# sencheng/CoBeL-RL

Measured on NVIDIA B200. Metric: agent-steps/sec incl. replay, higher is better.
Workload: dtype f64

## Files before the change

### cobel-rl_b200/csrc/dynaq.cu

```cuda
#include "warp_agent.cuh"

namespace {

constexpr int kWarpsPerCta = 4;

struct AgentSmem {
  int q, mr, mx, wm, rm, ptab, draws, vmax, pat, bytes;
  __host__ __device__ AgentSmem(int S, int A, bool plain, bool tables = true, bool sums = false) {
    const bool eps_tab = plain && A <= 4;
    const int SA = tables ? S * A : 0;
    q = 0;
    mr = q + SA * 8;
    wm = mr + SA * 8;
    rm = wm + S * 4;
    mx = rm + S * 4;
    ptab = (mx + SA * 2 + 15) & ~15;
    draws = ptab + (eps_tab ? kEpsTabDoubles * 8 : 0);
    vmax = draws + (plain ? kSmemDraws * 8 : 0);
    pat = vmax + (sums ? S * 8 : 0);
    bytes = sums ? (pat + S + 15) & ~15 : vmax;
  }
};

struct WorldSmem {
  int rew, succ, starts, term, bytes;
  __host__ __device__ WorldSmem(int S, int A, int K) {
    rew = 0;
    succ = rew + S * 8;
    starts = succ + S * A * 4;
    term = starts + K * 4;
    bytes = (term + S + 15) & ~15;
  }
};

template <int A, bool PLAIN, bool HBM = false, bool SUM = false>
__global__ void __launch_bounds__(kWarpsPerCta * 32, HBM ? 1 : 7) dynaq_warp_kernel(const __grid_constant__ CobelDynaQParams p) {
  static_assert(!(PLAIN && HBM), "the HBM path is the generic kernel");
  static_assert(!SUM || (PLAIN && A <= 4), "row summaries go with the tie-pattern table");
  extern __shared__ __align__(16) unsigned char smem[];
  const int S = p.world.n_states, K = p.world.n_starts, SA = S * A;
  const int lane = threadIdx.x & 31, warp = threadIdx.x >> 5;
  const WorldSmem wo(HBM ? 0 : S, A, HBM ? 0 : K);
  constexpr bool kEpsTab = PLAIN && A <= 4;
  const AgentSmem ao(S, A, PLAIN, !HBM, SUM);

  double* rew_s = reinterpret_cast<double*>(smem + wo.rew);
  int32_t* succ_s = reinterpret_cast<int32_t*>(smem + wo.succ);
  int32_t* starts_s = reinterpret_cast<int32_t*>(smem + wo.starts);
  uint8_t* term_s = smem + wo.term;
  if constexpr (!HBM) {
    for (int e = threadIdx.x; e < SA; e += blockDim.x) succ_s[e] = p.world.succ[e];
    for (int e = threadIdx.x; e < S; e += blockDim.x) { rew_s[e] = p.world.reward[e]; term_s[e] = p.world.terminal[e]; }
    for (int e = threadIdx.x; e < K; e += blockDim.x) starts_s[e] = p.world.starts[e];
    __syncthreads();
  }
  auto w_succ = [&](int sa) -> int { if constexpr (HBM) return __ldg(p.world.succ + sa); else return succ_s[sa]; };
  auto w_rew = [&](int x) -> double { if constexpr (HBM) return __ldg(p.world.reward + x); else return rew_s[x]; };
  auto w_term = [&](int x) -> int { if constexpr (HBM) return __ldg(p.world.terminal + x); else return term_s[x]; };
  auto w_start = [&](int k) -> int { if constexpr (HBM) return __ldg(p.world.starts + k); else return starts_s[k]; };

  const int64_t n = (int64_t)blockIdx.x * blockDim.x / 32 + warp;
  if (n >= p.n_agents) return;

  unsigned char* blk = smem + wo.bytes + (size_t)warp * ao.bytes;
  const size_t g0 = (size_t)n * SA;
  double* Q = HBM ? p.Q + g0 : reinterpret_cast<double*>(blk + ao.q);
  double* Mr = HBM ? p.Mr + g0 : reinterpret_cast<double*>(blk + ao.mr);
  uint16_t* Mx = reinterpret_cast<uint16_t*>(blk + ao.mx);
  int32_t* Msg = p.Ms + g0;
  int32_t* Mtg = p.Mt + g0;
  uint32_t* wm = reinterpret_cast<uint32_t*>(blk + ao.wm);
  uint32_t* rm = reinterpret_cast<uint32_t*>(blk + ao.rm);
  auto m_next = [&](int i, int& s2, int& nt) {
    if constexpr (HBM) { s2 = Msg[i]; nt = Mtg[i] ? 1 : 0; }
    else { const uint16_t v = Mx[i]; s2 = v & 0x7FFF; nt = v >> 15; }
  };
  auto m_set = [&](int i, int s2, int nt) {
    if constexpr (HBM) { Msg[i] = s2; Mtg[i] = nt; }
    else Mx[i] = (uint16_t)(s2 | (nt << 15));
  };

  if constexpr (!HBM) {
    for (int e = lane; e < SA; e += 32) {
      Q[e] = p.Q[g0 + e];
      Mr[e] = p.Mr[g0 + e];
      Mx[e] = (uint16_t)(p.Ms[g0 + e] | ((p.Mt[g0 + e] ? 1 : 0) << 15));
    }
  }
  __syncwarp();

  for (int e = lane; e < S; e += 32) { wm[e] = 0; rm[e] = 0; }
  double* V = reinterpret_cast<double*>(blk + ao.vmax);
  uint8_t* P = blk + ao.pat;
  if constexpr (SUM)
    for (int e = lane; e < S; e += 32) refresh_row_summary<A>(Q, V, P, e);
  typename WindowFor<PLAIN>::type win; win.init(p.stream, n, (uint64_t)p.stream.draw_count[n]);
  win.attach(reinterpret_cast<double*>(blk + ao.draws));
  const double lr = p.lr[n], gamma = p.gamma[n], mlr = p.mem_lr[n];
  PolicyTab pt; pt.init(p.policy.kind, p.policy.param[n], lane);
  double* ptab = reinterpret_cast<double*>(blk + ao.ptab);
  if constexpr (kEpsTab) eps_cdf_table_init<A>(ptab, pt, lane);
  const uint8_t* amask = (!PLAIN && p.action_mask) ? p.action_mask + n * p.mask_agent_stride : nullptr;
  const int B = PLAIN ? 32 : p.batch;
  const bool learn = PLAIN || p.learn != 0;
  const bool step_replay = PLAIN || (learn && !p.no_replay && !p.episodic_replay);
  const bool trial_replay = !PLAIN && learn && !p.no_replay && p.episodic_replay;
  const CobelTrace& tr = p.trace;
  int64_t nsteps = 0, nrep = 0, ncalls = 0;
  int flags = 0;

  auto replay = [&]() {
    for (int b0 = 0; b0 < B; b0 += 32) {
      const int nb = B - b0 < 32 ? B - b0 : 32;
      win.ensure(nb, lane);
      const bool active = lane < nb;
      const double u = win.peek(active ? lane : 0);
      win.advance(nb);
      int rs = 0, ra = 0, rs2 = 0, rnt = 0;
      double rr = 0.0;
      if (active) {
        const int i = draw_integer(u, SA);
        rs = i / A; ra = i - rs * A;
        rr = Mr[i];
        m_next(i, rs2, rnt);
        if (!PLAIN && tr.replay_idx) {
          if (nrep + lane < tr.replay_cap) tr.replay_idx[n * tr.replay_cap + nrep + lane] = i;
          else flags |= COBEL_FLAG_TRACE_OVERFLOW;
        }
      }
      td_batch_level_parallel<A>(Q, wm, rm, S, lane, active, rs, ra, rr, rs2, rnt, lr, gamma);
      nrep += nb;
    }
    if (!PLAIN && tr.replay_len && lane == 0) {
      if (ncalls < tr.replay_calls_cap) tr.replay_len[n * tr.replay_calls_cap + ncalls] = B;
      else flags |= COBEL_FLAG_TRACE_OVERFLOW;
    }
    ++ncalls;
  };

  for (int trial = 0; trial < p.trials; ++trial) {
    win.ensure(3 + (step_replay && B <= 32 ? B : 0), lane);
    int s = w_start(draw_integer(win.next(), K));
    double treward = 0.0;
    int step = 0;
    if constexpr (PLAIN) {
      for (;; ++step) {
        win.ensure(34, lane);
        const int i = draw_integer(win.peek(1 + lane), SA);
        double rr = Mr[i];
        int rs2, rnt;
        m_next(i, rs2, rnt);
        int a;
        if constexpr (SUM) {
          a = select_action_eps_pattern<A>(P[s], ptab, win.next(), lane);
        } else {
          double row[A];
          load_row<A>(Q + s * A, row);
          if constexpr (kEpsTab) a = select_action_eps_tab<A>(row, ptab, win.next(), lane);
          else a = select_action_warp<A, COBEL_POLICY_EPS_GREEDY>(row, (1u << A) - 1u, pt, win.next(), lane);
        }
        const int sa = s * A + a;
        const int s2 = w_succ(sa);
        const double r = w_rew(s2);
        const int end = w_term(s2);
        const int nt = 1 - end;
        const double m0 = Mr[sa];
        const double m1 = xadd(m0, xmul(mlr, xsub(r, m0)));
        double row2[A];
        if constexpr (!SUM) load_row<A>(Q + s2 * A, row2);
        const double q = Q[sa];
        const double g = nt ? gamma : 0.0;
        double td = xadd(r, xmul(g, SUM ? V[s2] : row_max<A>(row2)));
        td = xsub(td, q);
        const double qn = xadd(q, xmul(lr, td));
        if (i == sa) { rr = m1; rs2 = s2; rnt = nt; }
        const int rs = i / A, ra = i - rs * A;
        __syncwarp();
        if (lane == 0) {
          Mr[sa] = m1;
          m_set(sa, s2, nt);
          Q[sa] = qn;
          if (SUM && __double_as_longlong(qn) != __double_as_longlong(q)) refresh_row_summary<A>(Q, V, P, s);
        }
        __syncwarp();
        td_batch_level_parallel<A, SUM>(Q, wm, rm, S, lane, true, rs, ra, rr, rs2, rnt, lr, gamma, nullptr, nullptr, V, P);
        win.advance(32);
        ++nsteps;
        treward = xadd(treward, r);
        if (end || step + 1 == p.steps) break;
        s = s2;
      }
    } else for (;; ++step) {
      win.ensure(2 + (step_replay && B <= 32 ? B : 0), lane);
      double row[A];
      load_row<A>(Q + s * A, row);
      uint32_t mask = (1u << A) - 1u;
      if (amask) {
        mask = 0;
#pragma unroll
        for (int a = 0; a < A; ++a) mask |= (amask[s * A + a] ? 1u : 0u) << a;
      }
      const int a = select_action_warp<A>(row, mask, pt, win.next(), lane);
      const int s2 = p.world.tp_off ? stochastic_successor(p.world, s * A + a, win.next()) : w_succ(s * A + a);
      const double r = w_rew(s2);
      const int end = w_term(s2);
      const int nt = 1 - end;
      if (tr.step_sa && lane == 0) {
        if (nsteps < tr.step_cap) { tr.step_sa[n * tr.step_cap + nsteps] = s * A + a; if (tr.step_next) tr.step_next[n * tr.step_cap + nsteps] = s2; }
        else flags |= COBEL_FLAG_TRACE_OVERFLOW;
      }
      ++nsteps;
      if (learn) {
        const double m0 = Mr[s * A + a];
        const double m1 = xadd(m0, xmul(mlr, xsub(r, m0)));
        double row2[A];
        load_row<A>(Q + s2 * A, row2);
        const double q = Q[s * A + a];
        const double g = nt ? gamma : 0.0;
        double td = xadd(r, xmul(g, row_max<A>(row2)));
        td = xsub(td, q);
        const double qn = xadd(q, xmul(lr, td));
        if (tr.step_td && lane == 0) {
          if (nsteps <= tr.step_cap) tr.step_td[n * tr.step_cap + nsteps - 1] = td;
          else flags |= COBEL_FLAG_TRACE_OVERFLOW;
        }
        __syncwarp();
        if (lane == 0) {
          Mr[s * A + a] = m1;
          m_set(s * A + a, s2, nt);
          Q[s * A + a] = qn;
        }
        __syncwarp();
      }
      s = s2;
      if (step_replay) replay();
      treward = xadd(treward, r);
      if (end || step + 1 == p.steps) break;
    }
    if (lane == 0) {
      tr.trial_steps[n * p.trials + trial] = step;
      tr.trial_reward[n * p.trials + trial] = treward;
    }
    if (trial_replay) replay();
  }

  __syncwarp();
  if (learn && !HBM) {
    for (int e = lane; e < SA; e += 32) {
      p.Q[g0 + e] = Q[e];
      p.Mr[g0 + e] = Mr[e];
      p.Ms[g0 + e] = Mx[e] & 0x7FFF;
      p.Mt[g0 + e] = Mx[e] >> 15;
    }
  }
  flags = __reduce_or_sync(kFull, flags);
  if (lane == 0) {
    p.stream.draw_count[n] = (int64_t)win.position();
    tr.n_steps[n] += nsteps;
    tr.n_replay[n] += PLAIN ? nsteps * 32 : nrep;
    if (tr.flags && flags) tr.flags[n] |= flags;
  }
}


constexpr int kPairWarps = 2;
constexpr int kRing = 128;

struct PairSmem {
  int q, mr, mx, wm, rm, ptab, ring, bytes;
  __host__ __device__ PairSmem(int S, int A) {
    const int SA = S * A;
    q = 0;
    mr = q + SA * 8;
    wm = mr + SA * 8;
    rm = wm + S * 4;
    mx = rm + S * 4;
    ptab = (mx + SA * 2 + 15) & ~15;
    ring = ptab + kEpsTabDoubles * 8;
    bytes = ring + kRing * 8;
  }
};

template <int A>
__global__ void __launch_bounds__(kPairWarps * 32, 14) dynaq_pair_kernel(const __grid_constant__ CobelDynaQParams p) {
  static_assert(A <= 4, "tie-pattern table");
  extern __shared__ __align__(16) unsigned char smem[];
  const int S = p.world.n_states, K = p.world.n_starts, SA = S * A;
  const int lane = threadIdx.x & 31, warp = threadIdx.x >> 5, half = lane >> 4, h = lane & 15;
  const WorldSmem wo(S, A, K);
  const PairSmem ao(S, A);
  double* rew_s = reinterpret_cast<double*>(smem + wo.rew);
  int32_t* succ_s = reinterpret_cast<int32_t*>(smem + wo.succ);
  int32_t* starts_s = reinterpret_cast<int32_t*>(smem + wo.starts);
  uint8_t* term_s = smem + wo.term;
  for (int e = threadIdx.x; e < SA; e += blockDim.x) succ_s[e] = p.world.succ[e];
  for (int e = threadIdx.x; e < S; e += blockDim.x) { rew_s[e] = p.world.reward[e]; term_s[e] = p.world.terminal[e]; }
  for (int e = threadIdx.x; e < K; e += blockDim.x) starts_s[e] = p.world.starts[e];
  __syncthreads();

  const int64_t n = ((int64_t)blockIdx.x * kPairWarps + warp) * 2 + half;
  const bool mine = n < p.n_agents;
  const int64_t nn = mine ? n : p.n_agents - 1;
  unsigned char* blk = smem + wo.bytes + (size_t)(warp * 2 + half) * ao.bytes;
  const size_t g0 = (size_t)nn * SA;
  double* Q = reinterpret_cast<double*>(blk + ao.q);
  double* Mr = reinterpret_cast<double*>(blk + ao.mr);
  uint16_t* Mx = reinterpret_cast<uint16_t*>(blk + ao.mx);
  uint32_t* wm = reinterpret_cast<uint32_t*>(blk + ao.wm);
  uint32_t* rm = reinterpret_cast<uint32_t*>(blk + ao.rm);
  double* ptab = reinterpret_cast<double*>(blk + ao.ptab);
  double* ring = reinterpret_cast<double*>(blk + ao.ring);
  for (int e = h; e < SA; e += 16) {
    Q[e] = mine ? p.Q[g0 + e] : 0.0;
    Mr[e] = mine ? p.Mr[g0 + e] : 0.0;
    Mx[e] = mine ? (uint16_t)(p.Ms[g0 + e] | ((p.Mt[g0 + e] ? 1 : 0) << 15)) : (uint16_t)0;
  }
  for (int e = h; e < S; e += 16) { wm[e] = 0; rm[e] = 0; }
  for (int e = h; e < kRing; e += 16) ring[e] = 0.0;
  const double lr = p.lr[nn], gamma = p.gamma[nn], mlr = p.mem_lr[nn];
  {
    const double eps = p.policy.param[nn];
    const int pat = h & ((1 << A) - 1), k = __popc(pat);
    const double base = xdiv(eps, (double)A);
    const double tie = xdiv(xsub(1.0, eps), (double)(k > 0 ? k : 1));
    const double top = xadd(base, tie), low = xadd(base, 0.0);
    double cdf[A];
    double c = (pat & 1) ? top : low;
    cdf[0] = c;
#pragma unroll
    for (int a = 1; a < A; ++a) { c = xadd(c, (pat >> a & 1) ? top : low); cdf[a] = c; }
    if (c != 1.0) {
#pragma unroll
      for (int a = 0; a < A; ++a) cdf[a] = xdiv(cdf[a], c);
    }
    if (h > 0 && h < (1 << A)) {
#pragma unroll
      for (int a = 0; a < 4; ++a) ptab[pat * 4 + a] = a < A ? cdf[a] : 2.0;
    }
  }
  const uint64_t agent = (uint64_t)(p.stream.agent_id_base + nn);
  const uint32_t key0 = (uint32_t)p.stream.seed, key1 = (uint32_t)(p.stream.seed >> 32);
  const uint64_t pos0 = (uint64_t)p.stream.draw_count[nn];
  uint64_t gblk = (pos0 & ~31ull) >> 1;
  int wr = 0;
  int rd = (int)(pos0 & 31ull);
  int avail = -rd;
  const CobelTrace& tr = p.trace;
  bool live = mine && p.trials > 0;
  bool fresh = true;
  int s = 0, step = 0, trial = 0;
  int nsteps = 0;
  double treward = 0.0;
  __syncwarp();

  while (__any_sync(kFull, live)) {
    for (;;) {
      const bool need = live && avail < 34;
      if (!__any_sync(kFull, need)) break;
      const uint64_t b = gblk + (uint64_t)h;
      uint32_t o[4];
      philox4x32_10((uint32_t)b, (uint32_t)(b >> 32), (uint32_t)agent, (uint32_t)(agent >> 32), key0, key1, o);
      if (need) {
        reinterpret_cast<double2*>(ring)[(wr >> 1) + h] = make_double2(u53(o[0], o[1]), u53(o[2], o[3]));
        gblk += 16; wr = (wr + 32) & (kRing - 1); avail += 32;
      }
    }
    __syncwarp();
    if (fresh) {
      if (live) { s = starts_s[draw_integer(ring[rd], K)]; rd = (rd + 1) & (kRing - 1); --avail; }
      fresh = false; step = 0; treward = 0.0;
    }
    double row[A];
    load_row<A>(Q + s * A, row);
    const double ua = ring[rd];
    int a;
    {
      const double m = row_max<A>(row);
      uint32_t ties = 0;
#pragma unroll
      for (int x = 0; x < A; ++x) ties |= (row[x] == m ? 1u : 0u) << x;
      const double edge = ptab[ties * 4 + (h & 3)];
      const unsigned bal = __ballot_sync(kFull, h < A - 1 && edge <= ua);
      a = __popc((bal >> (half * 16)) & 0xFFFFu);
    }
    const int sa = s * A + a;
    const int s2 = succ_s[sa];
    const double r = rew_s[s2];
    const int end = term_s[s2];
    const int nt = 1 - end;
    {
      const double m0 = Mr[sa];
      const double m1 = xadd(m0, xmul(mlr, xsub(r, m0)));
      double row2[A];
      load_row<A>(Q + s2 * A, row2);
      const double q = Q[sa];
      const double g = nt ? gamma : 0.0;
      double td = xadd(r, xmul(g, row_max<A>(row2)));
      td = xsub(td, q);
      const double qn = xadd(q, xmul(lr, td));
      __syncwarp();
      if (live && h == 0) {
        Mr[sa] = m1;
        Mx[sa] = (uint16_t)(s2 | (nt << 15));
        Q[sa] = qn;
      }
      __syncwarp();
    }
#pragma unroll 1
    for (int b0 = 0; b0 < 32; b0 += 16) {
      const double u = ring[(rd + 1 + b0 + h) & (kRing - 1)];
      const int i = draw_integer(u, SA);
      const int rs = i / A, ra = i - rs * A;
      const double rr = Mr[i];
      const uint16_t v = Mx[i];
      td_batch_level_parallel<A>(Q, wm, rm, S, lane, live, rs, ra, rr, v & 0x7FFF, v >> 15, lr, gamma);
    }
    {
      const bool fin = end || step + 1 == p.steps;
      const double tw = xadd(treward, r);
      if (live && fin && h == 0) {
        tr.trial_steps[n * p.trials + trial] = step;
        tr.trial_reward[n * p.trials + trial] = tw;
      }
      const int adv = live ? 33 : 0;
      rd = (rd + adv) & (kRing - 1); avail -= adv;
      nsteps += live ? 1 : 0;
      treward = tw;
      trial += (live && fin) ? 1 : 0;
      fresh = fin;
      step = step + 1;
      s = s2;
      live = live && trial < p.trials;
    }
  }

  __syncwarp();
  if (mine) {
    for (int e = h; e < SA; e += 16) {
      p.Q[g0 + e] = Q[e];
      p.Mr[g0 + e] = Mr[e];
      p.Ms[g0 + e] = Mx[e] & 0x7FFF;
      p.Mt[g0 + e] = Mx[e] >> 15;
    }
    if (h == 0) {
      p.stream.draw_count[n] = (int64_t)(gblk * 2) - (int64_t)avail;
      tr.n_steps[n] += nsteps;
      tr.n_replay[n] += (int64_t)nsteps * 32;
    }
  }
}

template <int A>
int launch(const CobelDynaQParams& p, cudaStream_t st) {
  const int S = p.world.n_states, K = p.world.n_starts;
  const WorldSmem wo(S, A, K);
  const bool plain = !p.action_mask && !p.world.tp_off && !p.trace.step_sa && !p.trace.step_td && !p.trace.replay_idx &&
                     !p.trace.replay_len &&
                     p.policy.kind == COBEL_POLICY_EPS_GREEDY && p.learn && !p.no_replay && !p.episodic_replay &&
                     p.batch == 32 && !p.stream.user_stream;
  const AgentSmem ao(S, A, plain);
  const size_t sm = (size_t)wo.bytes + (size_t)kWarpsPerCta * ao.bytes;
  const unsigned grid = (unsigned)((p.n_agents + kWarpsPerCta - 1) / kWarpsPerCta);
  if (sm > kMaxSmem) {
    const AgentSmem go(S, A, false, false);
    int warps = kWarpsPerCta;
    while (warps > 1 && (size_t)warps * go.bytes > kMaxSmem) warps >>= 1;
    const size_t smg = (size_t)warps * go.bytes;
    COBEL_REQUIRE(smg <= kMaxSmem, COBEL_EUNSUPPORTED,
                  "Dyna-Q: the replay's dependency masks of %d states do not fit in shared memory (%zu bytes)", S, smg);
    return launch_kernel(dynaq_warp_kernel<A, false, true>, (unsigned)((p.n_agents + warps - 1) / warps), warps * 32, smg, st, p);
  }
  if constexpr (A <= 4) {
    const PairSmem po(S, A);
    const size_t smp = (size_t)wo.bytes + (size_t)kPairWarps * 2 * po.bytes;
    static const int n_sm = [] { int d = 0, v = 148; if (cudaGetDevice(&d) == cudaSuccess) cudaDeviceGetAttribute(&v, cudaDevAttrMultiProcessorCount, d); return v; }();
    if (plain && p.n_agents >= (int64_t)2 * 7 * kWarpsPerCta * n_sm && smp <= kMaxSmem && S <= 0x7FFF) {
      const int64_t per_cta = kPairWarps * 2;
      return launch_kernel(dynaq_pair_kernel<A>, (unsigned)((p.n_agents + per_cta - 1) / per_cta), kPairWarps * 32, smp, st, p);
    }
    const size_t sms = (size_t)wo.bytes + (size_t)kWarpsPerCta * AgentSmem(S, A, true, true, true).bytes;
    if (plain && sms <= kMaxSmem)
      return launch_kernel(dynaq_warp_kernel<A, true, false, true>, grid, kWarpsPerCta * 32, sms, st, p);
  }
  return launch_kernel(plain ? dynaq_warp_kernel<A, true> : dynaq_warp_kernel<A, false>, grid, kWarpsPerCta * 32, sm,
                       st, p);
}

}

extern "C" int cobel_dynaq_run(const CobelDynaQParams* pp, void* stream) {
  COBEL_REQUIRE(pp != nullptr, COBEL_EINVAL, "null params");
  const CobelDynaQParams& p = *pp;
  int rc = cobel_validate_common(p.n_agents, p.world, p.stream, p.policy, p.trace, p.trials, p.steps);
  if (rc) return rc;
  COBEL_REQUIRE(p.Q && p.Mr && p.Ms && p.Mt && p.lr && p.gamma && p.mem_lr, COBEL_EINVAL, "agent tables missing");
  COBEL_REQUIRE(p.batch >= 0, COBEL_EINVAL, "batch must be >= 0");
  if (p.trials == 0) return COBEL_OK;
  cudaStream_t st = reinterpret_cast<cudaStream_t>(stream);
  COBEL_DISPATCH_A(p.world.n_actions, return launch<A>(p, st));
}
```

### cobel-rl_b200/csrc/warp_agent.cuh

```cuda
#pragma once
#include "common.cuh"

constexpr unsigned kFull = 0xffffffffu;

COBEL_DEV double shfl_f64(double v, int src) {
  int lo = __double2loint(v), hi = __double2hiint(v);
  lo = __shfl_sync(kFull, lo, src);
  hi = __shfl_sync(kFull, hi, src);
  return __hiloint2double(hi, lo);
}

COBEL_DEV double shfl_f64_up(double v, int delta) {
  int lo = __double2loint(v), hi = __double2hiint(v);
  lo = __shfl_up_sync(kFull, lo, delta);
  hi = __shfl_up_sync(kFull, hi, delta);
  return __hiloint2double(hi, lo);
}

COBEL_DEV double shfl_f64_xor(double v, int m) {
  int lo = __double2loint(v), hi = __double2hiint(v);
  lo = __shfl_xor_sync(kFull, lo, m);
  hi = __shfl_xor_sync(kFull, hi, m);
  return __hiloint2double(hi, lo);
}

template <int A>
COBEL_DEV void load_row(const double* r, double (&v)[A]) {
  if constexpr (A % 2 == 0) {
#pragma unroll
    for (int x = 0; x < A; x += 2) {
      const double2 t = *reinterpret_cast<const double2*>(r + x);
      v[x] = t.x; v[x + 1] = t.y;
    }
  } else {
#pragma unroll
    for (int x = 0; x < A; ++x) v[x] = r[x];
  }
}

COBEL_DEV int stochastic_successor(const CobelWorld& w, int sa, double u) {
  const int lo = __ldg(w.tp_off + sa), hi = __ldg(w.tp_off + sa + 1);
  double tot = 0.0;
  for (int j = lo; j < hi; ++j) tot = xadd(tot, __ldg(w.tp_prob + j));
  double c = 0.0;
  for (int j = lo; j < hi; ++j) {
    c = xadd(c, __ldg(w.tp_prob + j));
    if (xdiv(c, tot) > u) return __ldg(w.tp_next + j);
  }
  return __ldg(w.tp_next + hi - 1);
}

static __device__ __noinline__ double2 philox_pair_shared(uint64_t b, uint64_t agent, uint32_t key0, uint32_t key1) {
  uint32_t o[4];
  philox4x32_10((uint32_t)b, (uint32_t)(b >> 32), (uint32_t)agent, (uint32_t)(agent >> 32), key0, key1, o);
  return make_double2(u53(o[0], o[1]), u53(o[2], o[3]));
}

template <bool MAYBE_USER, bool SMALL_CODE = false>
struct DrawWindowT {
  uint64_t agent;
  uint32_t key0, key1;
  uint64_t base;
  int off;
  int cap;
  double ua, ub;
  const double* user;
  int64_t user_len;

  COBEL_DEV void init(const CobelStream& s, int64_t local_agent, uint64_t k) {
    agent = (uint64_t)(s.agent_id_base + local_agent);
    key0 = (uint32_t)s.seed; key1 = (uint32_t)(s.seed >> 32);
    user = (MAYBE_USER && s.user_stream) ? s.user_stream + local_agent * s.user_stream_len : nullptr;
    user_len = s.user_stream_len;
    base = k; off = 0; cap = 0;
    ua = ub = 0.0;
  }
  COBEL_DEV uint64_t position() const { return base + (uint64_t)off; }
  COBEL_DEV void ensure(int need, int lane) {
    if ((MAYBE_USER && user) || off + need <= cap) return;
    const uint64_t k = base + (uint64_t)off;
    base = k & ~1ull; off = (int)(k & 1ull); cap = 64;
    const uint64_t b = (base >> 1) + lane;
    if constexpr (SMALL_CODE) {
      const double2 d = philox_pair_shared(b, agent, key0, key1);
      ua = d.x; ub = d.y;
    } else {
      uint32_t o[4];
      philox4x32_10((uint32_t)b, (uint32_t)(b >> 32), (uint32_t)agent, (uint32_t)(agent >> 32), key0, key1, o);
      ua = u53(o[0], o[1]); ub = u53(o[2], o[3]);
    }
  }
  COBEL_DEV double peek(int ahead) const {
    if (MAYBE_USER && user) {
      const uint64_t kk = base + (uint64_t)(off + ahead);
      return kk < (uint64_t)user_len ? user[kk] : 0.0;
    }
    const int slot = off + ahead;
    const double a = shfl_f64(ua, slot >> 1), b = shfl_f64(ub, slot >> 1);
    return (slot & 1) ? b : a;
  }
  COBEL_DEV void advance(int n) { off += n; }
  COBEL_DEV double next() { const double u = peek(0); ++off; return u; }
  COBEL_DEV void attach(double*) {}
};
using DrawWindow = DrawWindowT<true>;

constexpr int kSmemDraws = 256;
template <int NDRAWS>
struct SmemDrawWindowT {
  uint64_t agent;
  uint32_t key0, key1;
  uint64_t base;
  int off;
  int cap;
  double* buf;

  COBEL_DEV void attach(double* b) { buf = b; }
  COBEL_DEV void init(const CobelStream& s, int64_t local_agent, uint64_t k) {
    agent = (uint64_t)(s.agent_id_base + local_agent);
    key0 = (uint32_t)s.seed; key1 = (uint32_t)(s.seed >> 32);
    base = k; off = 0; cap = 0;
  }
  COBEL_DEV uint64_t position() const { return base + (uint64_t)off; }
  COBEL_DEV void ensure(int need, int lane) {
    if (off + need <= cap) return;
    const uint64_t k = base + (uint64_t)off;
    base = k & ~1ull; off = (int)(k & 1ull); cap = NDRAWS;
    __syncwarp();
#pragma unroll
    for (int j = 0; j < NDRAWS / 64; ++j) {
      const uint64_t b = (base >> 1) + (uint64_t)(j * 32 + lane);
      uint32_t o[4];
      philox4x32_10((uint32_t)b, (uint32_t)(b >> 32), (uint32_t)agent, (uint32_t)(agent >> 32), key0, key1, o);
      reinterpret_cast<double2*>(buf)[j * 32 + lane] = make_double2(u53(o[0], o[1]), u53(o[2], o[3]));
    }
    __syncwarp();
  }
  COBEL_DEV double peek(int ahead) const { return buf[off + ahead]; }
  COBEL_DEV void advance(int n) { off += n; }
  COBEL_DEV double next() { return buf[off++]; }
};
using SmemDrawWindow = SmemDrawWindowT<kSmemDraws>;
template <bool PLAIN, int NDRAWS = kSmemDraws> struct WindowFor { using type = DrawWindowT<true>; };
template <int NDRAWS> struct WindowFor<true, NDRAWS> { using type = SmemDrawWindowT<NDRAWS>; };

struct PolicyTab {
  int kind;
  double par;
  double q_par;
  double q_om;
  COBEL_DEV void init(int kind_, double par_, int lane) {
    kind = kind_; par = par_;
    q_par = xdiv(par_, (double)(lane + 1));
    q_om = xdiv(xsub(1.0, par_), (double)(lane + 1));
  }
};

template <int A, int KIND = -1>
COBEL_DEV int select_action_warp(const double (&v)[A], uint32_t mask, const PolicyTab& pt, double u, int lane) {
  const int kind = KIND >= 0 ? KIND : pt.kind;
  constexpr uint32_t kAll = (1u << A) - 1u;
  double m;
  int nv = A;
  if (mask == kAll) {
    m = row_max<A>(v);
  } else {
    nv = __popc(mask);
    m = -__longlong_as_double(0x7FF0000000000000ll);
#pragma unroll
    for (int a = 0; a < A; ++a) m = (mask >> a & 1u) ? xmax(m, v[a]) : m;
  }
  double p[A];
  if (kind == COBEL_POLICY_SOFTMAX) {
    double sum = 0.0;
#pragma unroll
    for (int a = 0; a < A; ++a) {
      p[a] = 0.0;
      if (mask >> a & 1u) { p[a] = exp(xmul(xsub(v[a], m), pt.par)); sum = xadd(sum, p[a]); }
    }
    if (A == 8 && mask == kAll) sum = np_sum<A>(p);
#pragma unroll
    for (int a = 0; a < A; ++a)
      if (mask >> a & 1u) p[a] = xdiv(p[a], sum);
  } else {
    uint32_t ties = 0;
#pragma unroll
    for (int a = 0; a < A; ++a) ties |= (v[a] == m ? 1u : 0u) << a;
    ties &= mask;
    const int k = __popc(ties);
    const double tie = shfl_f64(pt.q_om, k - 1);
    if (kind == COBEL_POLICY_EPS_GREEDY) {
      const double base = shfl_f64(pt.q_par, nv - 1);
      const double top = xadd(base, tie), low = xadd(base, 0.0);
#pragma unroll
      for (int a = 0; a < A; ++a)
        p[a] = (mask >> a & 1u) ? ((ties >> a & 1u) ? top : low) : 0.0;
    } else {
      const int d = nv - k > 1 ? nv - k : 1;
      const double expl = shfl_f64(pt.q_par, d - 1);
      const double top = xadd(tie, 0.0), low = xadd(0.0, expl);
#pragma unroll
      for (int a = 0; a < A; ++a)
        p[a] = (mask >> a & 1u) ? ((ties >> a & 1u) ? top : low) : 0.0;
    }
  }
  double c = p[0], mine = p[0];
#pragma unroll
  for (int a = 1; a < A; ++a) { c = xadd(c, p[a]); if (lane == a) mine = c; }
  if (c != 1.0) mine = xdiv(mine, c);
  const bool le = (lane < A - 1) && (mine <= u);
  return __popc(__ballot_sync(kFull, le));
}

constexpr int kEpsTabDoubles = 64;
template <int A>
COBEL_DEV void eps_cdf_table_init(double* tab, const PolicyTab& pt, int lane) {
  static_assert(A <= 4, "tie-pattern table is built for at most 4 actions");
  const int pat = lane & ((1 << A) - 1);
  const int k = __popc(pat);
  const double base = shfl_f64(pt.q_par, A - 1);
  const double tie = shfl_f64(pt.q_om, k > 0 ? k - 1 : 0);
  const double top = xadd(base, tie), low = xadd(base, 0.0);
  double cdf[A];
  double c = (pat & 1) ? top : low;
  cdf[0] = c;
#pragma unroll
  for (int a = 1; a < A; ++a) { c = xadd(c, (pat >> a & 1) ? top : low); cdf[a] = c; }
  if (c != 1.0) {
#pragma unroll
    for (int a = 0; a < A; ++a) cdf[a] = xdiv(cdf[a], c);
  }
  if (lane > 0 && lane < (1 << A)) {
#pragma unroll
    for (int a = 0; a < 4; ++a) tab[pat * 4 + a] = a < A ? cdf[a] : 2.0;
  }
  __syncwarp();
}
template <int A>
COBEL_DEV uint32_t tie_pattern(const double (&v)[A], double m) {
  uint32_t ties = 0;
#pragma unroll
  for (int a = 0; a < A; ++a) ties |= (v[a] == m ? 1u : 0u) << a;
  return ties;
}
template <int A>
COBEL_DEV int select_action_eps_pattern(uint32_t ties, const double* tab, double u, int lane) {
  const double mine = tab[ties * 4 + (lane & 3)];
  return __popc(__ballot_sync(kFull, lane < A - 1 && mine <= u));
}
template <int A>
COBEL_DEV int select_action_eps_tab(const double (&v)[A], const double* tab, double u, int lane) {
  return select_action_eps_pattern<A>(tie_pattern<A>(v, row_max<A>(v)), tab, u, lane);
}

template <int A>
COBEL_DEV void refresh_row_summary(const double* Q, double* V, uint8_t* P, int s) {
  double row[A];
  load_row<A>(Q + s * A, row);
  const double m = row_max<A>(row);
  V[s] = m;
  P[s] = (uint8_t)tie_pattern<A>(row, m);
}

template <int A, bool SUM = false>
COBEL_DEV void td_batch_level_parallel(double* Q, uint32_t* wm, uint32_t* rm, int S, int lane, bool active,
                                       int s, int a, double r, int s2, int nt, double lr, double gamma,
                                       const uint8_t* mbits = nullptr, double* td_out = nullptr,
                                       double* V = nullptr, uint8_t* P = nullptr) {
  static_assert(!SUM || A <= 4, "row summaries hold a tie pattern of at most 4 actions");
  const double g = nt ? gamma : 0.0;
  auto evaluate = [&](double& q, bool from_summary) -> double {
    double mx;
    if (SUM && from_summary) {
      q = Q[s * A + a];
      mx = V[s2];
    } else {
      double row[A];
      load_row<A>(Q + s2 * A, row);
      q = Q[s * A + a];
      if (mbits) {
        const uint32_t mb = mbits[s2];
        mx = -__longlong_as_double(0x7FF0000000000000ll);
#pragma unroll
        for (int x = 0; x < A; ++x) mx = (mb >> x & 1u) ? xmax(mx, row[x]) : mx;
      } else {
        mx = row_max<A>(row);
      }
    }
    double td = xadd(r, xmul(g, mx));
    td = xsub(td, q);
    if (td_out) *td_out = td;
    return xadd(q, xmul(lr, td));
  };
  double qn = 0.0;
  bool null = true;
  if (active) {
    double q;
    qn = evaluate(q, true);
    null = __double_as_longlong(qn) == __double_as_longlong(q);
  }
  unsigned bad = __ballot_sync(kFull, !null);
  if (bad == 0) return;

  const unsigned below = (1u << lane) - 1u;
  if (active) {
    atomicOr(&wm[s], 1u << lane);
    atomicOr(&rm[s2], 1u << lane);
  }
  unsigned same_a = 0;
#pragma unroll
  for (int x = 0; x < A; ++x) {
    const unsigned bx = __ballot_sync(kFull, active && a == x);
    same_a = a == x ? bx : same_a;
  }
  __syncwarp();
  unsigned raw = 0, dep = 0;
  if (active) {
    raw = (wm[s2] | (wm[s] & same_a)) & below;
    dep = raw | (rm[s] & below);
  }
  __syncwarp();
  if (active) { wm[s] = 0; rm[s2] = 0; }
  for (;;) {
    const bool valid = (raw & bad) == 0;
    const unsigned b = __ballot_sync(kFull, !(valid && null));
    if (b == bad) break;
    bad = b;
  }
  dep &= bad;
  unsigned done = ~bad;
  for (bool first = true; done != kFull; first = false) {
    const bool ready = !(done >> lane & 1u) && (dep & ~done) == 0;
    const unsigned R = __ballot_sync(kFull, ready);
    if (ready) {
      double q;
      Q[s * A + a] = first ? qn : evaluate(q, false);
    }
    __syncwarp();
    done |= R;
  }
  if constexpr (SUM) {
    if (bad >> lane & 1u) refresh_row_summary<A>(Q, V, P, s);
    __syncwarp();
  }
}
```

### profiles/row_summaries.py

```python
import os
import sys

import numpy as np

sys.path.insert(0, os.path.dirname(os.path.dirname(os.path.abspath(__file__))))
sys.path.insert(0, os.path.dirname(os.path.abspath(__file__)))
from oracle import tabular as tb
from oracle.philox import LazyStream
from cobel_rl_b200.misc.gridworld_tools import make_gridworld
from step_overlap import BATCH, EPS, GAMMA, LR, MEM_LR, SEED, bits, rounds, td_value

CASES = ('steps', 'online_refresh', 'online_self_loop', 'max_changed', 'pattern_changed', 'nonnull_batches',
         'kept_lanes', 'refreshed_states', 'round_same_state')


def xmax(a, b):
    return b if a < b else a


def row_max(row):
    if len(row) == 4:
        return xmax(xmax(row[0], row[1]), xmax(row[2], row[3]))
    m = row[0]
    for x in row[1:]:
        m = xmax(m, x)
    return m


def summary(row):
    m = row_max(row)
    return m, sum(1 << a for a in range(len(row)) if row[a] == m)


def summary_step(W, st, V, P, s, step, steps, rng, n):
    S, A = W['S'], W['A']
    Q, Mr, Ms, Mt = st['Q'], st['Mr'], st['Ms'], st['Mt']
    pattern = np.array([(P[s] >> x) & 1 for x in range(A)], dtype=np.float64)
    a = tb.draw_categorical(tb.action_probs(('eps', EPS), pattern), rng.next())
    s2, r, end = tb.env_step(W, s, a)
    nt, fin = 1 - end, bool(end or step + 1 == steps)
    Mr[s, a] += MEM_LR * (r - Mr[s, a]); Ms[s, a] = s2; Mt[s, a] = nt
    q = Q[s, a]
    td = r
    td += GAMMA * nt * V[s2]
    td -= q
    qn = q + LR * td
    Q[s, a] = qn
    if bits(qn) != bits(q):
        n['online_refresh'] += 1
        n['online_self_loop'] += s2 == s
        m, p = summary(Q[s])
        n['max_changed'] += bits(m) != bits(V[s])
        n['pattern_changed'] += p != P[s]
        V[s], P[s] = m, p
    items, spec, null = [], [], []
    for i in [tb.draw_integer(rng.next(), S * A) for _ in range(BATCH)]:
        rs, ra = divmod(i, A)
        items.append((rs, ra, int(Ms[rs, ra])))
        spec.append(td_value(np.array([V[items[-1][2]]]), Q[rs, ra], Mr[rs, ra], Mt[rs, ra]))
        null.append(bits(spec[-1]) == bits(Q[rs, ra]))
    if not all(null):
        valid = []
        for j, (rs, ra, x2) in enumerate(items):
            valid.append(all(valid[i] and null[i] for i in range(j)
                             if items[i][0] == x2 or items[i][:2] == (rs, ra)))
        kept = [not (v and z) for v, z in zip(valid, null)]
        for d, lanes in enumerate(rounds(items, kept)):
            states = [items[j][0] for j in lanes]
            n['round_same_state'] += len(states) - len(set(states))
            vals = [spec[j] if d == 0 else td_value(Q[items[j][2]], Q[items[j][0], items[j][1]],
                                                    Mr[items[j][0], items[j][1]], Mt[items[j][0], items[j][1]])
                    for j in lanes]
            for j, v in zip(lanes, vals):
                Q[items[j][0], items[j][1]] = v
        refreshed = {items[j][0] for j in range(BATCH) if kept[j]}
        n['nonnull_batches'] += 1
        n['kept_lanes'] += sum(kept)
        n['refreshed_states'] += len(refreshed)
        for x in refreshed:
            V[x], P[x] = summary(Q[x])
    n['steps'] += 1
    return s2, fin


def run(W, seed, agent, trials, steps, n=None, k0=1, Q0=None):
    n = n if n is not None else dict.fromkeys(CASES, 0)
    S, A = W['S'], W['A']
    ref, sm = tb.dynaq_init(S, A), tb.dynaq_init(S, A)
    if Q0 is not None:
        ref['Q'][:], sm['Q'][:] = Q0, Q0
    V = np.zeros(S)
    P = np.zeros(S, dtype=np.int64)
    for x in range(S):
        V[x], P[x] = summary(sm['Q'][x])
    rr, rk = tb.Draws(LazyStream(seed, agent), k0), tb.Draws(LazyStream(seed, agent), k0)
    for _ in range(trials):
        s = tb.env_reset(W, rr)
        assert tb.env_reset(W, rk) == s
        for step in range(steps):
            a = tb.select_action(('eps', EPS), ref['Q'][s], None, rr)
            s2, r, end = tb.env_step(W, s, a)
            ref['Mr'][s, a] += MEM_LR * (r - ref['Mr'][s, a]); ref['Ms'][s, a] = s2; ref['Mt'][s, a] = 1 - end
            tb._td_update(ref['Q'], s, a, r, s2, 1 - end, LR, GAMMA)
            for i in [tb.draw_integer(rr.next(), S * A) for _ in range(BATCH)]:
                rs, ra = divmod(i, A)
                tb._td_update(ref['Q'], rs, ra, ref['Mr'][rs, ra], int(ref['Ms'][rs, ra]), int(ref['Mt'][rs, ra]),
                              LR, GAMMA)
            s2k, fin = summary_step(W, sm, V, P, s, step, steps, rk, n)
            assert s2k == s2 and fin == bool(end or step + 1 == steps)
            assert rk.k == rr.k, 'draw count'
            for key in ('Q', 'Mr', 'Ms', 'Mt'):
                x, y = ref[key], sm[key]
                assert ((x.view(np.int64) == y.view(np.int64)) if x.dtype == np.float64 else (x == y)).all(), key
            for x in range(S):
                m, p = summary(sm['Q'][x])
                assert bits(V[x]) == bits(m) and P[x] == p, 'summary of state %d' % x
            s = s2
            if fin:
                break
    return n, sm, rk.k


def main():
    agents = [int(x) for x in sys.argv[1:]] or [0, 1]
    world = tb.compile_gridworld(make_gridworld(5, 5, terminals=[0], rewards=np.array([[0, 1]]), goals=[0]))
    n = dict.fromkeys(CASES, 0)
    for g in agents:
        run(world, SEED, g, 500, 50, n)
    st, nb = n['steps'], max(n['nonnull_batches'], 1)
    print('agents %s: %d steps, every step bit-identical to the sequential order, V and P exact after each' %
          (agents, st))
    print('  online refreshes (Q[s,a] changed)          %.4f per step (%d; %d self-loops s2 == s)' %
          (n['online_refresh'] / st, n['online_refresh'], n['online_self_loop']))
    print('    of which the row maximum changed         %d, the tie pattern changed %d' %
          (n['max_changed'], n['pattern_changed']))
    print('  batches with a kept update                 %.1f %% of steps' % (100 * n['nonnull_batches'] / st))
    print('    kept lanes per such batch                %.2f' % (n['kept_lanes'] / nb))
    print('    distinct refreshed states per batch      %.2f' % (n['refreshed_states'] / nb))
    print('  round lanes writing a state another lane of the round writes  %d' % n['round_same_state'])


if __name__ == '__main__':
    main()
```

Measured before the change: 3.262 billion.

## Track per-entry fixed-point bits to skip quiet Dyna-Q steps in small worlds

Adds per-entry flags for the plain warp kernel. One flag records whether the Q entry is a bit-exact TD fixed point under the current row maxima, the other whether the memory entry is already at its fixed point. When the online (s,a) and all 32 replay entries are fixed, the whole update and replay batch is skipped. The flags are kept current by refreshing touched entries and, whenever a row maximum changes, scanning all S*A entries that point to that state. The path is limited to S*A <= 128 and adds bookkeeping, ballots and extra shared memory on steps that are not quiet.

```diff
diff --git a/cobel-rl_b200/csrc/dynaq.cu b/cobel-rl_b200/csrc/dynaq.cu
--- a/cobel-rl_b200/csrc/dynaq.cu
+++ b/cobel-rl_b200/csrc/dynaq.cu
@@ -5,8 +5,8 @@
 constexpr int kWarpsPerCta = 4;
 
 struct AgentSmem {
-  int q, mr, mx, wm, rm, ptab, draws, vmax, pat, bytes;
-  __host__ __device__ AgentSmem(int S, int A, bool plain, bool tables = true, bool sums = false) {
+  int q, mr, mx, wm, rm, ptab, draws, vmax, pat, fz, vmark, bytes;
+  __host__ __device__ AgentSmem(int S, int A, bool plain, bool tables = true, bool sums = false, bool fix = false) {
     const bool eps_tab = plain && A <= 4;
     const int SA = tables ? S * A : 0;
     q = 0;
@@ -18,7 +18,9 @@
     draws = ptab + (eps_tab ? kEpsTabDoubles * 8 : 0);
     vmax = draws + (plain ? kSmemDraws * 8 : 0);
     pat = vmax + (sums ? S * 8 : 0);
-    bytes = sums ? (pat + S + 15) & ~15 : vmax;
+    fz = pat + (sums ? S : 0);
+    vmark = fz + (fix ? SA : 0);
+    bytes = sums ? (vmark + (fix ? S : 0) + 15) & ~15 : vmax;
   }
 };
 
@@ -33,16 +35,20 @@
   }
 };
 
-template <int A, bool PLAIN, bool HBM = false, bool SUM = false>
+constexpr int kRowSums = 1, kFixedPoints = 2;
+constexpr int kFixMaxEntries = 128;
+template <int A, bool PLAIN, bool HBM = false, int SUM = 0>
 __global__ void __launch_bounds__(kWarpsPerCta * 32, HBM ? 1 : 7) dynaq_warp_kernel(const __grid_constant__ CobelDynaQParams p) {
   static_assert(!(PLAIN && HBM), "the HBM path is the generic kernel");
   static_assert(!SUM || (PLAIN && A <= 4), "row summaries go with the tie-pattern table");
+  static_assert(SUM <= kFixedPoints, "summary level");
+  constexpr bool FIX = SUM == kFixedPoints;
   extern __shared__ __align__(16) unsigned char smem[];
   const int S = p.world.n_states, K = p.world.n_starts, SA = S * A;
   const int lane = threadIdx.x & 31, warp = threadIdx.x >> 5;
   const WorldSmem wo(HBM ? 0 : S, A, HBM ? 0 : K);
   constexpr bool kEpsTab = PLAIN && A <= 4;
-  const AgentSmem ao(S, A, PLAIN, !HBM, SUM);
+  const AgentSmem ao(S, A, PLAIN, !HBM, SUM != 0, FIX);
 
   double* rew_s = reinterpret_cast<double*>(smem + wo.rew);
   int32_t* succ_s = reinterpret_cast<int32_t*>(smem + wo.succ);
@@ -100,6 +106,28 @@
   PolicyTab pt; pt.init(p.policy.kind, p.policy.param[n], lane);
   double* ptab = reinterpret_cast<double*>(blk + ao.ptab);
   if constexpr (kEpsTab) eps_cdf_table_init<A>(ptab, pt, lane);
+  uint8_t* FZ = blk + ao.fz;
+  uint8_t* vmark = blk + ao.vmark;
+  auto f_refresh = [&](int e) {
+    const uint16_t x = Mx[e];
+    const double q = Q[e];
+    double td = xadd(Mr[e], xmul((x >> 15) ? gamma : 0.0, V[x & 0x7FFF]));
+    td = xsub(td, q);
+    const bool f = __double_as_longlong(xadd(q, xmul(lr, td))) == __double_as_longlong(q);
+    FZ[e] = (uint8_t)((FZ[e] & 2u) | (f ? 1u : 0u));
+  };
+  auto m_bit = [&](int e) -> uint32_t {
+    const double m0 = Mr[e];
+    const int t = w_succ(e);
+    const double r = w_rew(t);
+    return Mx[e] == (uint16_t)(t | (1 - w_term(t)) << 15) && __double_as_longlong(m0) == __double_as_longlong(r) &&
+           __double_as_longlong(xadd(m0, xmul(mlr, xsub(r, m0)))) == __double_as_longlong(m0) ? 2u : 0u;
+  };
+  if constexpr (FIX) {
+    for (int e = lane; e < S; e += 32) vmark[e] = 0;
+    for (int e = lane; e < SA; e += 32) { FZ[e] = (uint8_t)m_bit(e); f_refresh(e); }
+    __syncwarp();
+  }
   const uint8_t* amask = (!PLAIN && p.action_mask) ? p.action_mask + n * p.mask_agent_stride : nullptr;
   const int B = PLAIN ? 32 : p.batch;
   const bool learn = PLAIN || p.learn != 0;
@@ -150,6 +178,8 @@
         double rr = Mr[i];
         int rs2, rnt;
         m_next(i, rs2, rnt);
+        bool all_f = false;
+        if constexpr (FIX) all_f = __all_sync(kFull, FZ[i] & 1u);
         int a;
         if constexpr (SUM) {
           a = select_action_eps_pattern<A>(P[s], ptab, win.next(), lane);
@@ -164,26 +194,47 @@
         const double r = w_rew(s2);
         const int end = w_term(s2);
         const int nt = 1 - end;
-        const double m0 = Mr[sa];
-        const double m1 = xadd(m0, xmul(mlr, xsub(r, m0)));
-        double row2[A];
-        if constexpr (!SUM) load_row<A>(Q + s2 * A, row2);
-        const double q = Q[sa];
-        const double g = nt ? gamma : 0.0;
-        double td = xadd(r, xmul(g, SUM ? V[s2] : row_max<A>(row2)));
-        td = xsub(td, q);
-        const double qn = xadd(q, xmul(lr, td));
-        if (i == sa) { rr = m1; rs2 = s2; rnt = nt; }
-        const int rs = i / A, ra = i - rs * A;
-        __syncwarp();
-        if (lane == 0) {
-          Mr[sa] = m1;
-          m_set(sa, s2, nt);
-          Q[sa] = qn;
-          if (SUM && __double_as_longlong(qn) != __double_as_longlong(q)) refresh_row_summary<A>(Q, V, P, s);
+        if (!(FIX && all_f && FZ[sa] == 3u)) {
+          const double m0 = Mr[sa];
+          const double m1 = xadd(m0, xmul(mlr, xsub(r, m0)));
+          double row2[A];
+          if constexpr (!SUM) load_row<A>(Q + s2 * A, row2);
+          const double q = Q[sa];
+          const double g = nt ? gamma : 0.0;
+          double td = xadd(r, xmul(g, SUM ? V[s2] : row_max<A>(row2)));
+          td = xsub(td, q);
+          const double qn = xadd(q, xmul(lr, td));
+          if (i == sa) { rr = m1; rs2 = s2; rnt = nt; }
+          const int rs = i / A, ra = i - rs * A;
+          __syncwarp();
+          if (lane == 0) {
+            Mr[sa] = m1;
+            m_set(sa, s2, nt);
+            Q[sa] = qn;
+            if (SUM && __double_as_longlong(qn) != __double_as_longlong(q)) {
+              const double v0 = V[s];
+              refresh_row_summary<A>(Q, V, P, s);
+              if (FIX && __double_as_longlong(V[s]) != __double_as_longlong(v0)) vmark[s] = 1;
+            }
+            if constexpr (FIX) FZ[sa] = (uint8_t)((FZ[sa] & 1u) | m_bit(sa));
+          }
+          __syncwarp();
+          const unsigned kept = td_batch_level_parallel<A, SUM != 0>(Q, wm, rm, S, lane, true, rs, ra, rr, rs2, rnt, lr,
+                                                                     gamma, nullptr, nullptr, V, P, FIX ? vmark : nullptr);
+          if constexpr (FIX) {
+            __syncwarp();
+            f_refresh(kept >> lane & 1u ? i : sa);
+            if (kept == kFull && lane == 0) f_refresh(sa);
+            if (__any_sync(kFull, vmark[rs] | vmark[s])) {
+              for (int e = lane; e < SA; e += 32)
+                if (vmark[Mx[e] & 0x7FFF]) f_refresh(e);
+              __syncwarp();
+              vmark[rs] = 0;
+              vmark[s] = 0;
+            }
+            __syncwarp();
+          }
         }
-        __syncwarp();
-        td_batch_level_parallel<A, SUM>(Q, wm, rm, S, lane, true, rs, ra, rr, rs2, rnt, lr, gamma, nullptr, nullptr, V, P);
         win.advance(32);
         ++nsteps;
         treward = xadd(treward, r);
@@ -478,9 +529,13 @@
       const int64_t per_cta = kPairWarps * 2;
       return launch_kernel(dynaq_pair_kernel<A>, (unsigned)((p.n_agents + per_cta - 1) / per_cta), kPairWarps * 32, smp, st, p);
     }
+    if (plain && S * A <= kFixMaxEntries) {
+      const size_t smf = (size_t)wo.bytes + (size_t)kWarpsPerCta * AgentSmem(S, A, true, true, true, true).bytes;
+      return launch_kernel(dynaq_warp_kernel<A, true, false, kFixedPoints>, grid, kWarpsPerCta * 32, smf, st, p);
+    }
     const size_t sms = (size_t)wo.bytes + (size_t)kWarpsPerCta * AgentSmem(S, A, true, true, true).bytes;
     if (plain && sms <= kMaxSmem)
-      return launch_kernel(dynaq_warp_kernel<A, true, false, true>, grid, kWarpsPerCta * 32, sms, st, p);
+      return launch_kernel(dynaq_warp_kernel<A, true, false, kRowSums>, grid, kWarpsPerCta * 32, sms, st, p);
   }
   return launch_kernel(plain ? dynaq_warp_kernel<A, true> : dynaq_warp_kernel<A, false>, grid, kWarpsPerCta * 32, sm,
                        st, p);
diff --git a/cobel-rl_b200/csrc/warp_agent.cuh b/cobel-rl_b200/csrc/warp_agent.cuh
--- a/cobel-rl_b200/csrc/warp_agent.cuh
+++ b/cobel-rl_b200/csrc/warp_agent.cuh
@@ -263,10 +263,10 @@
 }
 
 template <int A, bool SUM = false>
-COBEL_DEV void td_batch_level_parallel(double* Q, uint32_t* wm, uint32_t* rm, int S, int lane, bool active,
-                                       int s, int a, double r, int s2, int nt, double lr, double gamma,
-                                       const uint8_t* mbits = nullptr, double* td_out = nullptr,
-                                       double* V = nullptr, uint8_t* P = nullptr) {
+COBEL_DEV unsigned td_batch_level_parallel(double* Q, uint32_t* wm, uint32_t* rm, int S, int lane, bool active,
+                                           int s, int a, double r, int s2, int nt, double lr, double gamma,
+                                           const uint8_t* mbits = nullptr, double* td_out = nullptr,
+                                           double* V = nullptr, uint8_t* P = nullptr, uint8_t* vmark = nullptr) {
   static_assert(!SUM || A <= 4, "row summaries hold a tie pattern of at most 4 actions");
   const double g = nt ? gamma : 0.0;
   auto evaluate = [&](double& q, bool from_summary) -> double {
@@ -300,7 +300,7 @@
     null = __double_as_longlong(qn) == __double_as_longlong(q);
   }
   unsigned bad = __ballot_sync(kFull, !null);
-  if (bad == 0) return;
+  if (bad == 0) return 0;
 
   const unsigned below = (1u << lane) - 1u;
   if (active) {
@@ -340,7 +340,17 @@
     done |= R;
   }
   if constexpr (SUM) {
-    if (bad >> lane & 1u) refresh_row_summary<A>(Q, V, P, s);
+    const bool kept = bad >> lane & 1u;
+    double v0 = 0.0;
+    if (vmark) {
+      if (kept) v0 = V[s];
+      __syncwarp();
+    }
+    if (kept) {
+      refresh_row_summary<A>(Q, V, P, s);
+      if (vmark && __double_as_longlong(V[s]) != __double_as_longlong(v0)) vmark[s] = 1;
+    }
     __syncwarp();
   }
-}
+  return bad;
+}
diff --git a/profiles/fixed_points.py b/profiles/fixed_points.py
--- /dev/null
+++ b/profiles/fixed_points.py
@@ -0,0 +1,148 @@
+import os
+import sys
+
+import numpy as np
+
+sys.path.insert(0, os.path.dirname(os.path.dirname(os.path.abspath(__file__))))
+sys.path.insert(0, os.path.dirname(os.path.abspath(__file__)))
+from oracle import tabular as tb
+from oracle.philox import LazyStream
+from cobel_rl_b200.misc.gridworld_tools import make_gridworld
+from step_overlap import BATCH, EPS, GAMMA, LR, MEM_LR, SEED, bits
+from row_summaries import CASES as SUM_CASES, summary, summary_step
+
+CASES = ('steps', 'quiet', 'sa_fixed_not_all_f', 'all_f_not_sa_fixed', 'nonquiet_nothing_written', 'entry_sa', 'entry_replay',
+         'scans', 'scan_states', 'scan_entries', 'recomputed', 'bit_flips')
+
+
+def f_bit(st, V, i):
+    q, r = st['Q'].flat[i], st['Mr'].flat[i]
+    g = GAMMA if st['Mt'].flat[i] else 0.0
+    td = r + g * V[int(st['Ms'].flat[i])]
+    td = td - q
+    return bits(q + LR * td) == bits(q)
+
+
+def m_bit(W, st, i):
+    t, r, end = tb.env_step(W, *divmod(i, W['A']))
+    m0 = st['Mr'].flat[i]
+    return (int(st['Ms'].flat[i]) == t and int(st['Mt'].flat[i] != 0) == 1 - end and bits(m0) == bits(r) and
+            bits(m0 + MEM_LR * (r - m0)) == bits(m0))
+
+
+def fz(W, st, V, i):
+    return int(f_bit(st, V, i)) | int(m_bit(W, st, i)) << 1
+
+
+def fixed_point_step(W, st, V, P, FZ, s, step, steps, rng, n):
+    S, A = W['S'], W['A']
+    Q, Mr, Ms, Mt = st['Q'], st['Mr'], st['Ms'], st['Mt']
+    idx = [tb.draw_integer(rng.u[rng.k + 1 + j], S * A) for j in range(BATCH)]
+    all_f = all(FZ[i] & 1 for i in idx)
+    pattern = np.array([(P[s] >> x) & 1 for x in range(A)], dtype=np.float64)
+    a = tb.draw_categorical(tb.action_probs(('eps', EPS), pattern), float(rng.u[rng.k]))
+    sa = s * A + a
+    z = FZ[sa] == 3
+    n['steps'] += 1
+    n['sa_fixed_not_all_f'] += z and not all_f
+    n['all_f_not_sa_fixed'] += all_f and not z
+    if z and all_f:
+        n['quiet'] += 1
+        rng.k += 1 + BATCH
+        s2, _, end = tb.env_step(W, s, a)
+        return s2, bool(end or step + 1 == steps)
+    old_sa = (bits(Mr.flat[sa]), int(Ms.flat[sa]), int(Mt.flat[sa]), bits(Q.flat[sa]))
+    marks = {'kept': set(), 'vmark': set()}
+    s2, fin = summary_step(W, st, V, P, s, step, steps, rng, dict.fromkeys(SUM_CASES, 0), marks)
+    wrote_sa = (bits(Mr.flat[sa]), int(Ms.flat[sa]), int(Mt.flat[sa]), bits(Q.flat[sa])) != old_sa
+    n['entry_sa'] += wrote_sa
+    FZ[sa] = (FZ[sa] & 1) | int(m_bit(W, st, sa)) << 1
+    redo = {sa} | marks['kept']
+    n['entry_replay'] += len(marks['kept'])
+    changed = marks['vmark']
+    assert changed <= {s} | {i // A for i in idx}
+    if changed:
+        n['scans'] += 1
+        n['scan_states'] += len(changed)
+        hits = [i for i in range(S * A) if int(Ms.flat[i]) in changed]
+        n['scan_entries'] += len(hits)
+        redo.update(hits)
+    n['nonquiet_nothing_written'] += not wrote_sa and not marks['kept']
+    for i in redo:
+        new = (FZ[i] & 2) | int(f_bit(st, V, i))
+        n['bit_flips'] += bin(new ^ int(FZ[i])).count('1')
+        FZ[i] = new
+    n['recomputed'] += len(redo)
+    return s2, fin
+
+
+def run(W, seed, agent, trials, steps, n=None, k0=1, init=None):
+    n = n if n is not None else dict.fromkeys(CASES, 0)
+    S, A = W['S'], W['A']
+    ref, fx = tb.dynaq_init(S, A), tb.dynaq_init(S, A)
+    for key, x0 in (init or {}).items():
+        ref[key][:], fx[key][:] = x0, x0
+    V = np.zeros(S)
+    P = np.zeros(S, dtype=np.int64)
+    for x in range(S):
+        V[x], P[x] = summary(fx['Q'][x])
+    FZ = np.array([fz(W, fx, V, i) for i in range(S * A)], dtype=np.int64)
+    rr, rk = tb.Draws(LazyStream(seed, agent), k0), tb.Draws(LazyStream(seed, agent), k0)
+    for _ in range(trials):
+        s = tb.env_reset(W, rr)
+        assert tb.env_reset(W, rk) == s
+        for step in range(steps):
+            a = tb.select_action(('eps', EPS), ref['Q'][s], None, rr)
+            s2, r, end = tb.env_step(W, s, a)
+            ref['Mr'][s, a] += MEM_LR * (r - ref['Mr'][s, a]); ref['Ms'][s, a] = s2; ref['Mt'][s, a] = 1 - end
+            tb._td_update(ref['Q'], s, a, r, s2, 1 - end, LR, GAMMA)
+            for i in [tb.draw_integer(rr.next(), S * A) for _ in range(BATCH)]:
+                rs, ra = divmod(i, A)
+                tb._td_update(ref['Q'], rs, ra, ref['Mr'][rs, ra], int(ref['Ms'][rs, ra]), int(ref['Mt'][rs, ra]),
+                              LR, GAMMA)
+            s2k, fin = fixed_point_step(W, fx, V, P, FZ, s, step, steps, rk, n)
+            assert s2k == s2 and fin == bool(end or step + 1 == steps)
+            assert rk.k == rr.k, 'draw count'
+            for key in ('Q', 'Mr', 'Ms', 'Mt'):
+                x, y = ref[key], fx[key]
+                assert ((x.view(np.int64) == y.view(np.int64)) if x.dtype == np.float64 else (x == y)).all(), key
+            for x in range(S):
+                m, p = summary(fx['Q'][x])
+                assert bits(V[x]) == bits(m) and P[x] == p, 'summary of state %d' % x
+            for i in range(S * A):
+                assert FZ[i] == fz(W, fx, V, i), 'fixed-point bits of entry %d' % i
+            s = s2
+            if fin:
+                break
+    return n, fx, rk.k
+
+
+def main():
+    agents = [int(x) for x in sys.argv[1:]] or [0, 1, 2, 3]
+    world = tb.compile_gridworld(make_gridworld(5, 5, terminals=[0], rewards=np.array([[0, 1]]), goals=[0]))
+    n = dict.fromkeys(CASES, 0)
+    for g in agents:
+        run(world, SEED, g, 500, 50, n)
+    st = n['steps']
+    nq = max(st - n['quiet'], 1)
+    print('agents %s: %d steps, every step bit-identical to the sequential order, V, P, F and M exact after each' %
+          (agents, st))
+    print('  quiet steps (F and M of (s,a), F of all 32 replay entries)   %.4f per step (%d)' %
+          (n['quiet'] / st, n['quiet']))
+    print('    (s,a) fixed but some replay F clear  %d;  all replay F set but (s,a) not fixed  %d' %
+          (n['sa_fixed_not_all_f'], n['all_f_not_sa_fixed']))
+    print('  maintenance after a non-quiet step (%d steps):' % (st - n['quiet']))
+    print('    nothing written                          %d' % n['nonquiet_nothing_written'])
+    print('    entry (s,a) written                      %.4f per step (%d)' % (n['entry_sa'] / st, n['entry_sa']))
+    print('    kept replay entries                      %.4f per step (%d)' % (n['entry_replay'] / st,
+                                                                             n['entry_replay']))
+    print('    scans over all S*A entries (V changed)   %.4f per step (%d; %.2f states, %.2f entries matched each)' %
+          (n['scans'] / st, n['scans'], n['scan_states'] / max(n['scans'], 1),
+           n['scan_entries'] / max(n['scans'], 1)))
+    print('    distinct entries recomputed              %.2f per non-quiet step (%d)' % (n['recomputed'] / nq,
+                                                                                     n['recomputed']))
+    print('    bit flips                                %.4f per step (%d)' % (n['bit_flips'] / st, n['bit_flips']))
+
+
+if __name__ == '__main__':
+    main()
diff --git a/profiles/row_summaries.py b/profiles/row_summaries.py
--- a/profiles/row_summaries.py
+++ b/profiles/row_summaries.py
@@ -32,7 +32,7 @@
     return m, sum(1 << a for a in range(len(row)) if row[a] == m)
 
 
-def summary_step(W, st, V, P, s, step, steps, rng, n):
+def summary_step(W, st, V, P, s, step, steps, rng, n, marks=None):
     S, A = W['S'], W['A']
     Q, Mr, Ms, Mt = st['Q'], st['Mr'], st['Ms'], st['Mt']
     pattern = np.array([(P[s] >> x) & 1 for x in range(A)], dtype=np.float64)
@@ -51,6 +51,8 @@
         n['online_self_loop'] += s2 == s
         m, p = summary(Q[s])
         n['max_changed'] += bits(m) != bits(V[s])
+        if marks is not None and bits(m) != bits(V[s]):
+            marks['vmark'].add(s)
         n['pattern_changed'] += p != P[s]
         V[s], P[s] = m, p
     items, spec, null = [], [], []
@@ -78,7 +80,12 @@
         n['kept_lanes'] += sum(kept)
         n['refreshed_states'] += len(refreshed)
         for x in refreshed:
-            V[x], P[x] = summary(Q[x])
+            m, p = summary(Q[x])
+            if marks is not None:
+                if bits(m) != bits(V[x]):
+                    marks['vmark'].add(x)
+                marks['kept'].update(items[j][0] * A + items[j][1] for j in range(BATCH) if kept[j])
+            V[x], P[x] = m, p
     n['steps'] += 1
     return s2, fin
 
```

New measurement: 3.321 billion, median of 6. 1.02x the previous value.
